# fabiocarrara/neural-ode-features

Measured on AMD Instinct MI355X. Metric: images/sec (fwd+adjoint) CIFAR-10 ODE-ResNet bs=128 at 1/2/4/8 GPU, higher is better.
Workload: dtype f32

## Files before the change

### neural-ode-features_amd/csrc/kernels_stem.hip

```cpp
#include "stem.h"

namespace node {

namespace {

typedef float f32x16 __attribute__((ext_vector_type(16)));
typedef __bf16 bf16x8 __attribute__((ext_vector_type(8)));
typedef __bf16 bf16x2 __attribute__((ext_vector_type(2)));
typedef float f32x2 __attribute__((ext_vector_type(2)));
typedef unsigned u32x4 __attribute__((ext_vector_type(4)));

__device__ __forceinline__ void split3(float x, bf16_t& h, bf16_t& m, bf16_t& l) {
  const __bf16 bh = (__bf16)x;
  const float r = x - (float)bh;
  const __bf16 bm = (__bf16)r;
  const float r2 = r - (float)bm;
  const __bf16 bl = (__bf16)r2;
  h = __builtin_bit_cast(bf16_t, bh);
  m = __builtin_bit_cast(bf16_t, bm);
  l = __builtin_bit_cast(bf16_t, bl);
}
__device__ __forceinline__ void split8(const float4& p, const float4& q, u32x4& hh, u32x4& mm, u32x4& ll) {
  const f32x2 v[4] = {{p.x, p.y}, {p.z, p.w}, {q.x, q.y}, {q.z, q.w}};
#pragma unroll
// ... 545 lines not shown
    if (a.dh) {
      *reinterpret_cast<float4*>(a.dh + o) = p0;
      *reinterpret_cast<float4*>(a.dh + o + 4) = p1;
    }
    if (a.dh3) {
      u32x4 hh, mm, ll;
      split8(p0, p1, hh, mm, ll);
      *reinterpret_cast<u32x4*>(a.dh3 + o) = hh;
      *reinterpret_cast<u32x4*>(a.dh3 + o + a.dh_plane) = mm;
      *reinterpret_cast<u32x4*>(a.dh3 + o + 2 * a.dh_plane) = ll;
    }
  }
}

__global__ __launch_bounds__(256) void k_stem_from_nchw(const float* __restrict__ src, float* __restrict__ dst, bf16_t* __restrict__ dst3,
                                                        size_t plane, int C, int HW) {
  __shared__ float tile[64][65];
  const int t = threadIdx.x;
  const int npb = (HW + 63) / 64, ncb = C / 64;
  const int n = blockIdx.x / (npb * ncb), rem = blockIdx.x - n * npb * ncb, cb = rem / npb, pb = rem - cb * npb;
  const int c0 = cb * 64, p0 = pb * 64;
  for (int idx = t; idx < 64 * 64; idx += 256) {
    const int cc = idx >> 6, pp = idx & 63;
    tile[cc][pp] = p0 + pp < HW ? src[((size_t)n * C + c0 + cc) * HW + p0 + pp] : 0.f;
  }
  __syncthreads();
  for (int idx = t; idx < 64 * 8; idx += 256) {
    const int pp = idx >> 3, q = idx & 7;
    if (p0 + pp >= HW) continue;
    float v[8];
#pragma unroll
    for (int k = 0; k < 8; ++k) v[k] = tile[8 * q + k][pp];
    const size_t o = ((size_t)n * HW + p0 + pp) * C + c0 + 8 * q;
    const float4 a0 = make_float4(v[0], v[1], v[2], v[3]), a1 = make_float4(v[4], v[5], v[6], v[7]);
    if (dst) {
      *reinterpret_cast<float4*>(dst + o) = a0;
      *reinterpret_cast<float4*>(dst + o + 4) = a1;
    }
    if (dst3) {
      u32x4 hh, mm, ll;
      split8(a0, a1, hh, mm, ll);
      *reinterpret_cast<u32x4*>(dst3 + o) = hh;
      *reinterpret_cast<u32x4*>(dst3 + o + plane) = mm;
      *reinterpret_cast<u32x4*>(dst3 + o + 2 * plane) = ll;
    }
  }
}

__global__ __launch_bounds__(256) void k_stem_split(const float* __restrict__ src, bf16_t* __restrict__ dst3, size_t plane, size_t n8) {
  const size_t i = (size_t)blockIdx.x * 256 + threadIdx.x;
  if (i >= n8) return;
  const float4 a0 = reinterpret_cast<const float4*>(src)[2 * i], a1 = reinterpret_cast<const float4*>(src)[2 * i + 1];
  u32x4 hh, mm, ll;
  split8(a0, a1, hh, mm, ll);
  *reinterpret_cast<u32x4*>(dst3 + 8 * i) = hh;
  *reinterpret_cast<u32x4*>(dst3 + 8 * i + plane) = mm;
  *reinterpret_cast<u32x4*>(dst3 + 8 * i + 2 * plane) = ll;
}

__global__ __launch_bounds__(256) void k_stem_to_nchw(const float* __restrict__ src, float* __restrict__ dst, int C, int HW) {
  __shared__ float tile[64][65];
  const int t = threadIdx.x;
  const int npb = (HW + 63) / 64, ncb = C / 64;
  const int n = blockIdx.x / (npb * ncb), rem = blockIdx.x - n * npb * ncb, cb = rem / npb, pb = rem - cb * npb;
  const int c0 = cb * 64, p0 = pb * 64;
// ... 23 lines not shown
    const float v = j.w[((size_t)co * j.Cin + ci) * j.taps + tap];
    bf16_t h, m, l;
    split3(v, h, m, l);
    const size_t of = ((size_t)tap * j.Cout + co) * j.Cin + ci, od = ((size_t)tap * j.Cin + ci) * j.Cout + co;
    j.wf[of] = h; j.wf[of + total] = m; j.wf[of + 2 * total] = l;
    j.wd[od] = h; j.wd[od + total] = m; j.wd[od + 2 * total] = l;
    return;
  }
  if (job == a.njobs) {
    if (a.w0t == nullptr || idx >= 28 * 64) return;
    const int k = (int)(idx / 64), co = (int)(idx % 64);
    a.w0t[idx] = k < a.k0 ? a.w0[co * a.k0 + k] : 0.f;
    return;
  }
  const int which = (int)(idx / 4096), e = (int)(idx % 4096);
  if (which >= a.nzero * 3) return;
  const int ten = which / 3, p = which - 3 * ten;
  if (e < a.zero_c[ten]) a.zero[ten][p * a.zero_plane[ten] + e] = 0;
}

__global__ __launch_bounds__(256) void k_stem_reduce(const SReduceArgs a) {
  __shared__ float part[4][64];
  int ji = 0;
  while (ji + 1 < a.njobs && blockIdx.x >= a.blk0[ji + 1]) ++ji;
  const SReduceJob& j = a.job[ji];
  const unsigned bx = blockIdx.x - a.blk0[ji];
  const int t = threadIdx.x;
  if (j.kind == 0) {
    const int co = bx / j.taps, tap = bx - co * j.taps;
    if (co >= j.Co) return;
// ... 107 lines not shown
}
void launch_stem_gn_bwd(const SGnArgs& a, hipStream_t s) {
  static bool attr[MAX_DEVICES] = {};
  allow_full_lds(reinterpret_cast<const void*>(k_stem_gn_bwd), attr);
  hipLaunchKernelGGL(k_stem_gn_bwd, dim3(a.N * (a.C / a.CB)), dim3(256), ((size_t)2 * a.HW * a.CB + 1024) * sizeof(float), s, a);
}

void launch_stem_prep(const SPrepArgs& a0, hipStream_t s) {
  SPrepArgs a = a0;
  unsigned at = 0;
  for (int i = 0; i < 6; ++i) {
    a.blk0[i] = at;
    if (i < a.njobs) at += (unsigned)(((size_t)a.job[i].taps * a.job[i].Cout * a.job[i].Cin + 255) / 256);
  }
  a.blk0[6] = at; at += (28 * 64 + 255) / 256;
  a.blk0[7] = at; at += (unsigned)(((size_t)a.nzero * 3 * 4096 + 255) / 256);
  a.blk0[8] = at;
  hipLaunchKernelGGL(k_stem_prep, dim3(at), dim3(256), 0, s, a);
}
void launch_stem_from_nchw(const float* src, float* dst_nhwc, bf16_t* dst3, size_t plane, int N, int C, int HW, hipStream_t s) {
  hipLaunchKernelGGL(k_stem_from_nchw, dim3(N * (C / 64) * ((HW + 63) / 64)), dim3(256), 0, s, src, dst_nhwc, dst3, plane, C, HW);
}
void launch_stem_split(const float* src, bf16_t* dst3, size_t plane, size_t n, hipStream_t s) {
  hipLaunchKernelGGL(k_stem_split, dim3((unsigned)((n / 8 + 255) / 256)), dim3(256), 0, s, src, dst3, plane, n / 8);
}
void launch_stem_to_nchw(const float* src_nhwc, float* dst, int N, int C, int HW, hipStream_t s) {
  hipLaunchKernelGGL(k_stem_to_nchw, dim3(N * (C / 64) * ((HW + 63) / 64)), dim3(256), 0, s, src_nhwc, dst, C, HW);
}
void launch_stem_reduce(const SReduceArgs& a0, hipStream_t s) {
  SReduceArgs a = a0;
  unsigned at = 0;
  for (int i = 0; i < a.njobs; ++i) {
    const SReduceJob& j = a.job[i];
    a.blk0[i] = at;
    at += (unsigned)(j.kind == 0 ? j.Co * j.taps : j.kind == 1 ? 64 : (2 * j.Co + 31) / 32);
  }
  a.blk0[a.njobs] = at;
  if (at == 0) return;
  hipLaunchKernelGGL(k_stem_reduce, dim3(at), dim3(256), 0, s, a);
// ... 4 lines not shown
```

### neural-ode-features_amd/csrc/kernels_w4.hip

```cpp
#include "wino4.h"
#include <cstdlib>
#include <cstring>

namespace node {

typedef float float16_t __attribute__((ext_vector_type(16)));
typedef __attribute__((address_space(3))) void* w4_lds_ptr_t;

#ifndef NODE_WT_STORES
#define NODE_WT_STORES 1
#endif
__device__ __forceinline__ void st_wt(float* p, float v) {
#if NODE_WT_STORES
  __hip_atomic_store(p, v, __ATOMIC_RELAXED, __HIP_MEMORY_SCOPE_AGENT);
#else
  *p = v;
#endif
}

__device__ __forceinline__ unsigned short w4_bf16_rne(float v) {
  const unsigned u = __builtin_bit_cast(unsigned, v);
  return (unsigned short)((u + 0x7FFFu + ((u >> 16) & 1u)) >> 16);
}
__device__ __forceinline__ float w4_bf16_f32(unsigned short b) { return __builtin_bit_cast(float, (unsigned)b << 16); }
// ... 1173 lines not shown
      }
      float* mrow = M + ((size_t)(rb * 8 + 2 * r4 + hi) * (gm.C >> 5) + 2 * ct + blk) * (36 * 128) + (size_t)scomp * 128 + l31;
      st_wt(mrow, s.x);
      st_wt(mrow + 32, s.y);
      st_wt(mrow + 64, s.z);
      st_wt(mrow + 96, s.w);
    }
  }
}



#endif

constexpr int W4SC_BLOCKS = 32;
__global__ __launch_bounds__(256) void k_w4_scales(W4ScaleJobs j, int nbig) {
  __shared__ float red[4];
  int job, part, parts;
  if ((int)blockIdx.x < nbig * W4SC_BLOCKS) {
    const int b = blockIdx.x / W4SC_BLOCKS;
    part = blockIdx.x - b * W4SC_BLOCKS; parts = W4SC_BLOCKS;
    job = j.bigjob[b];
  } else {
    job = 2 + ((int)blockIdx.x - nbig * W4SC_BLOCKS); part = 0; parts = 1;
  }
  const float* p = job < 2 ? j.w[job] : j.gb[job - 2];
  size_t n = job < 2 ? j.wn : (size_t)j.C;
  const bool big_vec = (job == 3 || job == 5) && j.vn[(job - 3) >> 1] != 0;
  if (big_vec) n = j.vn[(job - 3) >> 1];
  if (parts == 1 && big_vec) p = nullptr;
  float m = 0.f;
  if (p != nullptr) {
    const size_t i0 = (size_t)part * 256 + threadIdx.x, step = (size_t)parts * 256;
    if ((reinterpret_cast<uintptr_t>(p) & 15) == 0 && (n & 3) == 0) {
      const float4* q = reinterpret_cast<const float4*>(p);
      const size_t n4 = n >> 2;
      for (size_t i = i0; i < n4; i += 4 * step) {
        float4 v[4];
#pragma unroll
// ... 25 lines not shown
  }
  __hip_atomic_store(&sc->arrived, 0u, __ATOMIC_RELAXED, __HIP_MEMORY_SCOPE_AGENT);
  if (j.w[0] != nullptr) sc->e[W4_E_U1] = w4_scale_exp(3.49f * mx[0], 14);
  if (j.w[1] != nullptr) sc->e[W4_E_U2] = w4_scale_exp(3.49f * mx[1], 14);
  const float rm = sqrtf((float)j.gn_m);
  if (j.gb[0] != nullptr || j.gb[1] != nullptr) sc->e[W4_E_V1] = w4_scale_exp(49.f * (rm * mx[2] + mx[3]), 15);
  if (j.gb[2] != nullptr || j.gb[3] != nullptr) sc->e[W4_E_V2] = w4_scale_exp(49.f * (rm * mx[4] + mx[5]), 15);
}
void launch_w4_scales(const W4ScaleJobs& j_in, hipStream_t s) {
  W4ScaleJobs j = j_in;
  int nbig = 0;
  if (j.w[0] != nullptr) j.bigjob[nbig++] = 0;
  if (j.w[1] != nullptr) j.bigjob[nbig++] = 1;
  if (j.vn[0] != 0) j.bigjob[nbig++] = 3;
  if (j.vn[1] != 0) j.bigjob[nbig++] = 5;
  hipLaunchKernelGGL(k_w4_scales, dim3(nbig * W4SC_BLOCKS + 4), dim3(256), 0, s, j, nbig);
}

typedef _Float16 w4_f16x8 __attribute__((ext_vector_type(8)));
struct W4HStage { w4_u32x4 a[2][2], b[2][2]; };
struct W4HCursor { const w4_u32x4* a[2]; const w4_u32x4* b[2]; };
template <int NRB>
__device__ __forceinline__ void w4h_next(W4HStage& s, W4HCursor& cu) {
#pragma unroll
  for (int r = 0; r < NRB; ++r) {
    s.a[r][0] = cu.a[r][0];
    s.a[r][1] = cu.a[r][64];
    cu.a[r] += 128;
  }
#pragma unroll
  for (int c = 0; c < 2; ++c) {
// ... 1229 lines not shown
```

### neural-ode-features_amd/csrc/kernels_w4s.hip

```cpp
#include "wino4.h"
#include <cstring>

namespace node {

#ifndef W4S_THREADS_DEF
#define W4S_THREADS_DEF 128
#endif
constexpr int W4S_THREADS = W4S_THREADS_DEF;

#ifndef NODE_WT_STORES
#define NODE_WT_STORES 1
#endif
__device__ __forceinline__ void w4s_st_wt(float* p, float v) {
#if NODE_WT_STORES
  __hip_atomic_store(p, v, __ATOMIC_RELAXED, __HIP_MEMORY_SCOPE_AGENT);
#else
  *p = v;
#endif
}

template <int CTRL>
__device__ __forceinline__ float w4s_dpp(float v) {
  return __builtin_bit_cast(float, __builtin_amdgcn_update_dpp(0, __builtin_bit_cast(int, v), CTRL, 0xf, 0xf, true));
}
// ... 735 lines not shown
void launch_w4_input(const float* x_w4s, float* V, int N, int C, int Q, int Nv, hipStream_t s, const int* v_exp) {
  dim3 grid, block;
  w4s_grid(N, C, 1, Q, grid, block);
  if (Q == 1) hipLaunchKernelGGL(k_w4s_input<1>, grid, block, 0, s, x_w4s, V, C, Nv, v_exp);
  else hipLaunchKernelGGL(k_w4s_input<4>, grid, block, 0, s, x_w4s, V, C, Nv, v_exp);
}
void launch_w4_output(const float* M, float* y_w4s, int N, int C, int Q, hipStream_t s) {
  dim3 grid, block;
  w4s_grid(N, C, 1, Q, grid, block);
  if (Q == 1) hipLaunchKernelGGL(k_w4s_output<1>, grid, block, 0, s, M, y_w4s, C);
  else hipLaunchKernelGGL(k_w4s_output<4>, grid, block, 0, s, M, y_w4s, C);
}

__global__ __launch_bounds__(W4S_THREADS) void k_w4s_stem_in(const float* __restrict__ h, const float* __restrict__ gamma,
                                                             const float* __restrict__ beta, float eps, int cpg, float* __restrict__ xhat_s,
                                                             float* __restrict__ rstd, float* __restrict__ V, int C, int Nv) {
  W4Wave<1> wv;
  w4s_place(wv, C, nullptr, nullptr);
  const float* base = h + ((size_t)wv.n * 64 + (4 * wv.TY) * 8 + 4 * wv.TX) * C + wv.c;
  float y[4][4];
#pragma unroll
  for (int i = 0; i < 4; ++i)
#pragma unroll
    for (int j = 0; j < 4; ++j) y[i][j] = base[(size_t)(i * 8 + j) * C];
  float mean, rs;
  w4s_gn_stats(y, cpg, 1.0f / (float)(64 * cpg), eps, wv, mean, rs);
  const float gam = gamma[wv.c], bet = beta[wv.c];
  float xh[4][4], v[4][4];
#pragma unroll
  for (int i = 0; i < 4; ++i)
#pragma unroll
    for (int j = 0; j < 4; ++j) {
      xh[i][j] = (y[i][j] - mean) * rs;
      v[i][j] = fmaxf(fmaf(xh[i][j], gam, bet), 0.f);
    }
  const size_t f4 = ((size_t)wv.nv * (C >> 4) + wv.cb) * 256 + wv.lane;
#pragma unroll
  for (int i = 0; i < 4; ++i) w4s_st4(xhat_s, f4 + i * 64, xh[i]);
  if (wv.t == 0 && wv.c % cpg == 0) rstd[(size_t)wv.n * (C / cpg) + wv.c / cpg] = rs;
  w4s_put_v(v, wv, V, C, Nv);
}
__global__ __launch_bounds__(W4S_THREADS) void k_w4s_stem_out(const float* __restrict__ M, const float* __restrict__ res, float* __restrict__ out, int C) {
  W4Wave<1> wv;
  w4s_place(wv, C, nullptr, nullptr);
  float z[4][4];
  w4s_out_transform(w4s_m_ptr(M, wv, C), z);
  const float* rb = res + ((size_t)wv.n * 64 + (4 * wv.TY) * 8 + 4 * wv.TX) * C + wv.c;
  float* ob = out + ((size_t)wv.n * C + wv.c) * 64 + (4 * wv.TY) * 8 + 4 * wv.TX;
#pragma unroll
  for (int i = 0; i < 4; ++i) {
    float4 o;
    o.x = z[i][0] + rb[(size_t)(i * 8 + 0) * C];
    o.y = z[i][1] + rb[(size_t)(i * 8 + 1) * C];
    o.z = z[i][2] + rb[(size_t)(i * 8 + 2) * C];
    o.w = z[i][3] + rb[(size_t)(i * 8 + 3) * C];
    *reinterpret_cast<float4*>(ob + i * 8) = o;
  }
}
__global__ __launch_bounds__(W4S_THREADS) void k_w4s_stem_gin(const float* __restrict__ g, float* __restrict__ V, float* __restrict__ Z, int C, int Nv) {
  W4Wave<1> wv;
  w4s_place(wv, C, nullptr, nullptr);
  const float* gb = g + ((size_t)wv.n * C + wv.c) * 64 + (4 * wv.TY) * 8 + 4 * wv.TX;
  float v[4][4];
#pragma unroll
  for (int i = 0; i < 4; ++i) {
    const float4 q = *reinterpret_cast<const float4*>(gb + i * 8);
    v[i][0] = q.x; v[i][1] = q.y; v[i][2] = q.z; v[i][3] = q.w;
  }
  w4s_emit_z(v, wv.nv, Nv, C, wv.c, wv.t, Z);
  w4s_put_v(v, wv, V, C, Nv);
}
__global__ __launch_bounds__(256) void k_w4_du_to_dw(const float* __restrict__ dU, float* __restrict__ dW, int C) {
  const size_t CC = (size_t)C * C;
  const size_t idx = (size_t)blockIdx.x * 256 + threadIdx.x;
  if (idx >= CC) return;
  const int ci = (int)(idx / C), co = (int)(idx - (size_t)ci * C);
  float tq[6][3];
#pragma unroll
  for (int xi = 0; xi < 6; ++xi) {
    float u[6];
#pragma unroll
    for (int nu = 0; nu < 6; ++nu) u[nu] = dU[(size_t)(xi * 6 + nu) * CC + idx];
#pragma unroll
    for (int kw = 0; kw < 3; ++kw) {
      float sacc = 0.f;
// ... 8 lines not shown
  float* o = dW + ((size_t)co * C + ci) * 9;
#pragma unroll
  for (int kh = 0; kh < 3; ++kh)
#pragma unroll
    for (int kw = 0; kw < 3; ++kw) {
      float sacc = 0.f;
#pragma unroll
      for (int xi = 0; xi < 6; ++xi) {
        const float gq = (float)W4_G[xi][kh];
        if (gq != 0.f) sacc += gq * tq[xi][kw];
      }
      o[kh * 3 + kw] = sacc;
    }
}
void launch_w4s_stem_in(const float* h_nhwc, const float* gamma, const float* beta, float eps, int cpg, float* xhat_s, float* rstd, float* V,
                        int N, int C, int Nv, hipStream_t s) {
  dim3 grid, block;
  w4s_grid(N, C, cpg, 1, grid, block);
  hipLaunchKernelGGL(k_w4s_stem_in, grid, block, 0, s, h_nhwc, gamma, beta, eps, cpg, xhat_s, rstd, V, C, Nv);
}
void launch_w4s_stem_out(const float* M, const float* res_nhwc, float* out_nchw, int N, int C, hipStream_t s) {
  dim3 grid, block;
  w4s_grid(N, C, 1, 1, grid, block);
  hipLaunchKernelGGL(k_w4s_stem_out, grid, block, 0, s, M, res_nhwc, out_nchw, C);
}
void launch_w4s_stem_gin(const float* g_nchw, float* V, float* Z, int N, int C, int Nv, hipStream_t s) {
  dim3 grid, block;
  w4s_grid(N, C, 1, 1, grid, block);
  hipLaunchKernelGGL(k_w4s_stem_gin, grid, block, 0, s, g_nchw, V, Z, C, Nv);
}
void launch_w4_du_to_dw(const float* dU, float* dW, int C, hipStream_t s) {
  const size_t CC = (size_t)C * C;
  hipLaunchKernelGGL(k_w4_du_to_dw, dim3((unsigned)((CC + 255) / 256)), dim3(256), 0, s, dU, dW, C);
}

}
```

### neural-ode-features_amd/csrc/stem.h

```cpp
#pragma once
#include "node_internal.h"

namespace node {

typedef unsigned short bf16_t;

struct SConvArgs {
  const bf16_t* in;
  size_t in_plane;
  int zero_row;
  const bf16_t* w;
  size_t w_plane;
  float* out;
  const float* res;
  const float* bias;
  int accumulate;
  const bf16_t* w2;
  size_t w2_plane;
  float* out2;
  const bf16_t* in2;
  int N, IH, IW;
  int OH, OW;
  int Cin, Cout;
  int KH, KW, sshift, pad;
// ... 39 lines not shown
  size_t dh_plane;
  float* gpart;
  int N, HW, C, cpg, CB;
  float eps;
};
int stem_gn_cb(int HW, int C, int cpg);
void launch_stem_gn_fwd(const SGnArgs& a, hipStream_t s);
void launch_stem_gn_bwd(const SGnArgs& a, hipStream_t s);

struct SPrepJob { const float* w; bf16_t* wf; bf16_t* wd; int Cout, Cin, taps; };
struct SPrepArgs {
  SPrepJob job[6];
  int njobs;
  const float* w0; float* w0t; int k0;
  bf16_t* zero[10]; size_t zero_plane[10]; int zero_c[10]; int nzero;
  unsigned blk0[9];
};
void launch_stem_prep(const SPrepArgs& a, hipStream_t s);
void launch_stem_from_nchw(const float* src, float* dst_nhwc, bf16_t* dst3, size_t plane, int N, int C, int HW, hipStream_t s);
void launch_stem_to_nchw(const float* src_nhwc, float* dst, int N, int C, int HW, hipStream_t s);
void launch_stem_split(const float* src, bf16_t* dst3, size_t plane, size_t n , hipStream_t s);
struct SReduceJob { const float* slab; float* out; float* out2; int kind, ns, Co, Ci, taps; };
struct SReduceArgs { SReduceJob job[12]; int njobs; unsigned blk0[13]; };
void launch_stem_reduce(const SReduceArgs& a, hipStream_t s);

}
```

### neural-ode-features_amd/csrc/stem_api.hip

```cpp
#include "stem.h"
#include "wino4.h"
#include "../../include/node_hip.h"
#include <cstdarg>
#include <cstdio>
#include <cstring>

using namespace node;

namespace {

int failf(int code, const char* fmt, ...) {
  char buf[512];
  va_list ap;
  va_start(ap, fmt);
  vsnprintf(buf, sizeof(buf), fmt, ap);
  va_end(ap);
  return set_error(code, buf);
}

struct Bump {
  char* base;
  size_t off;
  explicit Bump(void* b) : base((char*)b), off(0) {}
  template <typename T>
// ... 56 lines not shown
struct StemPlan {
  int N, Cin0, H, W, F;
  int H0, W0, H1, W1, H2, W2, R0, R1, R2;
  float eps;
  float* w0t;
  Filt c1, c2, d1, c3, c4, d2;
  float *h0, *h1, *s1, *x1, *h3, *s2, *outn;
  Trip a0, a1, a2, a3;
  float* stats[4];
  float *da3, *da2, *da1, *da0, *dh0;
  Trip g3, dh3t, dx1t, dh1t;
  float* gpart[4];
  Wg w4, w3, w2, w1, w0;
  bool f4;
  bool f4_b16;
  float *xh4, *rs4, *Va, *Vg, *M4, *Z4, *dU4, *U4[2], *dh3n;
  unsigned short* Ub4[2];
  size_t bytes;
};

bool stem_takes_w4(const node_stem_shape* sh) {
  const char* e = getenv("NODE_TUNE_STEM_W4");
  if (e && atoi(e) == 0) return false;
  const int h2 = ((sh->h - 2 - 1) / 2 + 1 - 1) / 2 + 1, w2 = ((sh->w - 2 - 1) / 2 + 1 - 1) / 2 + 1;
  return h2 == 8 && w2 == 8 && sh->filters % 128 == 0 && sh->n % 8 == 0 && 16 % (sh->filters / 32) == 0;
}

StemPlan make_stem_plan(const node_stem_shape* sh, void* base) {
  StemPlan p;
  memset(&p, 0, sizeof(p));
  p.N = sh->n; p.Cin0 = sh->in_ch; p.H = sh->h; p.W = sh->w; p.F = sh->filters; p.eps = sh->eps;
  p.H0 = p.H - 2; p.W0 = p.W - 2;
  p.H1 = down2(p.H0); p.W1 = down2(p.W0);
  p.H2 = down2(p.H1); p.W2 = down2(p.W1);
  p.R0 = p.N * p.H0 * p.W0; p.R1 = p.N * p.H1 * p.W1; p.R2 = p.N * p.H2 * p.W2;
  const int F = p.F, G64 = 32, GF = F < 32 ? F : 32;
  Bump b(base);
  p.w0t = b.take<float>(28 * 64);
  p.c1 = take_filt(b, 64, 64, 9);
  p.c2 = take_filt(b, 64, 64, 9);
// ... 35 lines not shown
  p.w1 = take_wg(b, p.R1, 64, 64, 9, true);
  {
    int ns = p.R0 / 256;
    if (ns > 1024) ns = 1024;
    if (ns < 1) ns = 1;
    int rps = ((p.R0 + ns - 1) / ns + 7) & ~7;
    p.w0.rps = rps;
    p.w0.nsplit = (p.R0 + rps - 1) / rps;
    p.w0.slab = b.take<float>((size_t)p.w0.nsplit * 64 * 32);
    p.w0.slab2 = nullptr;
  }
  p.f4 = stem_takes_w4(sh);
  if (p.f4) {
    const int Nv = p.N;
    p.f4_b16 = w4_uses_bf16(Nv, F);
    p.xh4 = b.take<float>((size_t)p.R2 * F);
    p.rs4 = b.take<float>((size_t)p.N * GF);
    p.Va = b.take<float>(w4_v_elems(Nv, F));
    p.Vg = b.take<float>(w4_v_elems(Nv, F));
    p.M4 = b.take<float>(w4_v_elems(Nv, F));
    p.Z4 = b.take<float>(w4_z_elems(Nv, F));
    p.dU4 = b.take<float>((size_t)W4_COMPS * F * F);
    for (int i = 0; i < 2; ++i) {
      p.U4[i] = b.take<float>(w4_u_elems(F));
      p.Ub4[i] = b.take<unsigned short>(w4_ub_elems(F));
    }
    p.dh3n = b.take<float>((size_t)p.R2 * F);
  }
  p.bytes = b.off + 256;
  return p;
}

int check_stem_shape(const node_stem_shape* sh) {
  if (!sh) return failf(NODE_ERR_NULL, "shape is NULL");
  if (sh->n <= 0 || sh->in_ch <= 0 || sh->h < 5 || sh->w < 5 || sh->filters <= 0) return failf(NODE_ERR_SHAPE, "bad stem shape");
  if (sh->in_ch > 3) return failf(NODE_ERR_UNSUPPORTED, "the stem's first layer takes in_ch <= 3 (got %d)", sh->in_ch);
  if (sh->filters % 64 != 0) return failf(NODE_ERR_UNSUPPORTED, "the stem's kernels take filters %% 64 == 0 (got %d)", sh->filters);
  const size_t biggest = (size_t)sh->n * (sh->h - 2) * (sh->w - 2) * 64;
  if (biggest >= ((size_t)1 << 31)) return failf(NODE_ERR_UNSUPPORTED, "stem tensors must stay under 2^31 elements");
  if (stem_gn_cb((sh->h - 2) * (sh->w - 2), 64, 2) == 0)
    return failf(NODE_ERR_UNSUPPORTED, "the stem's GroupNorm passes hold (sample, 8 channels) blocks in LDS: images up to %d pixels "
                 "behind the first layer (got %d x %d)", 150 * 1024 / 64, sh->h - 2, sh->w - 2);
// ... 105 lines not shown
  if (rc != NODE_OK) return rc;
  if (!prm || !x || !out || !ws) return failf(NODE_ERR_NULL, "a required pointer is NULL");
  const float* const* pp = reinterpret_cast<const float* const*>(prm);
  for (int i = 0; i < 16; ++i)
    if (!pp[i]) return failf(NODE_ERR_NULL, "stem parameter %d is NULL", i);
  if (((uintptr_t)ws) & 255) return failf(NODE_ERR_ARG, "workspace must be 256-byte aligned");
  StemPlan p = make_stem_plan(shape, ws);
  if (ws_bytes < p.bytes) return failf(NODE_ERR_WORKSPACE, "stem workspace too small: %zu < %zu", ws_bytes, p.bytes);
  hipStream_t st = (hipStream_t)stream;
  const int N = p.N, F = p.F;

  SPrepArgs pa;
  memset(&pa, 0, sizeof(pa));
  const Filt* fl[6] = {&p.c1, &p.c2, &p.d1, &p.c3, &p.c4, &p.d2};
  const float* fw[6] = {prm->b1_c1_w, prm->b1_c2_w, prm->b1_ds_w, prm->b2_c1_w, prm->b2_c2_w, prm->b2_ds_w};
  for (int i = 0; i < 6; ++i) pa.job[i] = {fw[i], fl[i]->wf, fl[i]->wd, fl[i]->Cout, fl[i]->Cin, fl[i]->taps};
  pa.njobs = 6;
  pa.w0 = prm->conv0_w; pa.w0t = p.w0t; pa.k0 = 9 * p.Cin0;
  const Trip* tz[8] = {&p.a0, &p.a1, &p.a2, &p.a3, &p.g3, &p.dh3t, &p.dx1t, &p.dh1t};
  for (int i = 0; i < 8; ++i) {
    pa.zero[i] = tz[i]->p + (size_t)tz[i]->rows * tz[i]->C;
    pa.zero_plane[i] = tz[i]->plane;
    pa.zero_c[i] = tz[i]->C;
  }
  pa.nzero = 8;
  if (F > 4096) return failf(NODE_ERR_UNSUPPORTED, "filters > 4096");
  launch_stem_prep(pa, st);
  if ((rc = launch_ok("stem_prep")) != NODE_OK) return rc;

  launch_stem_conv0_fwd(x, p.w0t, prm->conv0_b, p.h0, N, p.Cin0, p.H, p.W, st);
  if ((rc = launch_ok("stem_conv0_fwd")) != NODE_OK) return rc;
  {
// ... 21 lines not shown
    if ((rc = launch_ok("stem_conv")) != NODE_OK) return rc;
  }
  {
    SGnArgs g = gn_args(p.x1, prm->b2_n1_w, prm->b2_n1_b, p.stats[2], N, p.H1 * p.W1, 64, p.eps);
    g.a3 = p.a2.p; g.a_plane = p.a2.plane;
    launch_stem_gn_fwd(g, st);
    if ((rc = launch_ok("stem_gn_fwd")) != NODE_OK) return rc;
  }
  {
    SConvArgs c = conv_fwd_args(p.a2, p.c3, p.h3, N, p.H1, p.W1, p.H2, p.W2, 3, 2, 1);
    c.w2 = p.d2.wf; c.w2_plane = p.d2.plane; c.out2 = p.s2;
    launch_stem_conv(c, st);
    if ((rc = launch_ok("stem_conv")) != NODE_OK) return rc;
  }
  if (p.f4) {
    W4PackJobs jobs;
    memset(&jobs, 0, sizeof(jobs));
    for (int i = 0; i < 2; ++i) {
      jobs.w[i] = prm->b2_c2_w; jobs.u[i] = p.U4[i]; jobs.ub[i] = p.f4_b16 ? p.Ub4[i] : nullptr; jobs.dgrad[i] = i; jobs.plain[i] = 1;
    }
    launch_w4_pack(jobs, 2, F, st);
    if ((rc = launch_ok("w4_pack")) != NODE_OK) return rc;
    launch_w4s_stem_in(p.h3, prm->b2_n2_w, prm->b2_n2_b, p.eps, F / 32, p.xh4, p.rs4, p.Va, N, F, N, st);
    if ((rc = launch_ok("w4s_stem_in")) != NODE_OK) return rc;
    launch_w4_gemm(p.Va, p.U4[0], p.M4, nullptr, N, F, st, p.f4_b16 ? p.Ub4[0] : nullptr);
    if ((rc = launch_ok("w4_gemm")) != NODE_OK) return rc;
    launch_w4s_stem_out(p.M4, p.s2, out, N, F, st);
    return launch_ok("node_stem_fwd");
  }
  {
    SGnArgs g = gn_args(p.h3, prm->b2_n2_w, prm->b2_n2_b, p.stats[3], N, p.H2 * p.W2, F, p.eps);
    g.a3 = p.a3.p; g.a_plane = p.a3.plane;
    launch_stem_gn_fwd(g, st);
    if ((rc = launch_ok("stem_gn_fwd")) != NODE_OK) return rc;
  }
  {
    SConvArgs c = conv_fwd_args(p.a3, p.c4, p.outn, N, p.H2, p.W2, p.H2, p.W2, 3, 1, 1);
    c.res = p.s2;
    launch_stem_conv(c, st);
    if ((rc = launch_ok("stem_conv")) != NODE_OK) return rc;
// ... 8 lines not shown
  w4_refresh_tuning();
  int rc = check_stem_shape(shape);
  if (rc != NODE_OK) return rc;
  if (!prm || !x || !grad_out || !gr || !ws) return failf(NODE_ERR_NULL, "a required pointer is NULL");
  const float* const* pp = reinterpret_cast<const float* const*>(prm);
  float* const* gp = reinterpret_cast<float* const*>(gr);
  for (int i = 0; i < 16; ++i)
    if (!pp[i] || !gp[i]) return failf(NODE_ERR_NULL, "stem parameter / gradient %d is NULL", i);
  if (((uintptr_t)ws) & 255) return failf(NODE_ERR_ARG, "workspace must be 256-byte aligned");
  StemPlan p = make_stem_plan(shape, ws);
  if (ws_bytes < p.bytes) return failf(NODE_ERR_WORKSPACE, "stem workspace too small: %zu < %zu", ws_bytes, p.bytes);
  hipStream_t st = (hipStream_t)stream;
  const int N = p.N, F = p.F;
  const int HW0 = p.H0 * p.W0, HW1 = p.H1 * p.W1, HW2 = p.H2 * p.W2;

  launch_stem_from_nchw(grad_out, nullptr, p.g3.p, p.g3.plane, N, F, HW2, st);
  if ((rc = launch_ok("stem_from_nchw")) != NODE_OK) return rc;
  if (p.f4) {
    launch_w4s_stem_gin(grad_out, p.Vg, p.Z4, N, F, N, st);
    if ((rc = launch_ok("w4s_stem_gin")) != NODE_OK) return rc;
    launch_w4_gemm(p.Vg, p.U4[1], p.M4, nullptr, N, F, st, p.f4_b16 ? p.Ub4[1] : nullptr);
    if ((rc = launch_ok("w4_gemm")) != NODE_OK) return rc;
    W4sArgs a;
    memset(&a, 0, sizeof(a));
    a.N = N; a.Q = 1; a.Nv = N; a.C = F; a.cpg = F / 32; a.eps = p.eps;
    a.h.M = p.M4; a.h.gamma = prm->b2_n2_w; a.h.beta = prm->b2_n2_b; a.h.xhat_s = p.xh4; a.h.rstd = p.rs4; a.h.osign = 1.f;
    a.h.gpart = p.gpart[3]; a.h.out_nhwc = p.dh3n;
    launch_w4s_pass(2, 0, a, st);
    if ((rc = launch_ok("w4s_pass")) != NODE_OK) return rc;
    launch_stem_split(p.dh3n, p.dh3t.p, p.dh3t.plane, (size_t)p.R2 * F, st);
    if ((rc = launch_ok("stem_split")) != NODE_OK) return rc;
    W4WgradArgs wa;
    memset(&wa, 0, sizeof(wa));
    wa.V1 = p.Va; wa.Z1 = p.Z4; wa.dU = p.dU4; wa.N = N; wa.C = F;
    launch_w4_wgrad(wa, st);
    if ((rc = launch_ok("w4_wgrad")) != NODE_OK) return rc;
    launch_w4_du_to_dw(p.dU4, gr->b2_c2_w, F, st);
    if ((rc = launch_ok("w4_du_to_dw")) != NODE_OK) return rc;
  } else {
    launch_stem_wgrad(wgrad_args(p.g3, nullptr, p.a3, p.w4, N, p.H2, p.W2, p.H2, p.W2, F, F, 3, 1, 1), st);
    if ((rc = launch_ok("stem_wgrad")) != NODE_OK) return rc;
    launch_stem_conv(conv_dgrad_args(p.g3, p.c4, p.da3, N, p.H2, p.W2, p.H2, p.W2, 3, 1, 1), st);
    if ((rc = launch_ok("stem_conv")) != NODE_OK) return rc;
    {
      SGnArgs g = gn_args(p.h3, prm->b2_n2_w, prm->b2_n2_b, p.stats[3], N, HW2, F, p.eps);
      g.da = p.da3; g.dh = nullptr; g.dh3 = p.dh3t.p; g.dh_plane = p.dh3t.plane; g.gpart = p.gpart[3];
      launch_stem_gn_bwd(g, st);
      if ((rc = launch_ok("stem_gn_bwd")) != NODE_OK) return rc;
    }
  }
// ... 146 lines not shown
```

### neural-ode-features_amd/csrc/wino4.h

```cpp
#pragma once
#include "node_internal.h"

namespace node {

constexpr int W4_COMPS = 36;

__device__ constexpr float W4_BT[6][6] = {{1.f, -1.5f, -2.f, 1.5f, 1.f, 0.f}, {0.f, -1.f, 0.5f, 2.5f, 1.f, 0.f},
                                          {0.f, 1.f, -2.5f, 0.5f, 1.f, 0.f},  {0.f, -2.f, -1.f, 2.f, 1.f, 0.f},
                                          {0.f, 0.5f, -1.f, -0.5f, 1.f, 0.f}, {0.f, 1.f, -1.5f, -2.f, 1.5f, 1.f}};
__device__ constexpr float W4_AT[4][6] = {{1.f, 1.f, 1.f, 1.f, 1.f, 0.f},
                                          {0.f, 1.f, -1.f, 0.5f, -2.f, 0.f},
                                          {0.f, 1.f, 1.f, 0.25f, 4.f, 0.f},
                                          {0.f, 1.f, -1.f, 0.125f, -8.f, 1.f}};
__device__ constexpr double W4_G[6][3] = {{1.0, 0.0, 0.0},
                                          {1.0 / 3, 1.0 / 3, 1.0 / 3},
                                          {-1.0 / 3, 1.0 / 3, -1.0 / 3},
                                          {-16.0 / 15, -8.0 / 15, -4.0 / 15},
                                          {1.0 / 15, -2.0 / 15, 4.0 / 15},
                                          {0.0, 0.0, 1.0}};

struct W4Geom {
  int N, C, RB, G8, R;
};
__host__ __device__ inline W4Geom w4_geom(int N, int C) {
// ... 37 lines not shown
    __hip_atomic_store(&sc->ovf, 0u, __ATOMIC_RELAXED, __HIP_MEMORY_SCOPE_AGENT);
    if (g > 0.f && g < INFINITY) sc->e[4] = w4_scale_exp(g, W4_G_TOP);
    if (ovf) sc->n_retry += 1;
  }
  return ovf;
}
void launch_w4_gscale(W4Scales* sc, hipStream_t s, int skew = 0);
constexpr int W4_E_U1 = 0, W4_E_U2 = 1, W4_E_V1 = 2, W4_E_V2 = 3, W4_E_G = 4;
struct W4ScaleJobs {
  const float* w[2];
  size_t wn;
  const float* gb[4];
  size_t vn[2];
  int C, gn_m;
  W4Scales* sc;
  int bigjob[4];
};
void launch_w4_scales(const W4ScaleJobs& j, hipStream_t s);
constexpr int W4_SLACK = 16 * 256;
__host__ __device__ inline size_t w4_v_elems(int N, int C) { return (size_t)W4_COMPS * 4 * N * C + W4_SLACK; }
__host__ __device__ inline size_t w4_u_elems(int C) { return (size_t)W4_COMPS * C * C + W4_SLACK; }

struct W4sHead {
  const float* M;
  const float* bias;
  const float* tmapS;
  EvalTime et;
  const float* gamma;
  const float* beta;
  float osign;
// ... 57 lines not shown

constexpr float W4_MIN_TOL = 0.99e-5f;
struct W4PackJobs { const float* w[4]; float* u[4]; unsigned short* ub[4]; int dgrad[4]; int plain[4]; unsigned* uh[4]; const int* uh_exp[4]; };
bool w4_uses_bf16(int N, int C);
__host__ __device__ inline size_t w4_ub_elems(int C) { return (size_t)W4_COMPS * C * C * 3 + 8 * 1536; }
void launch_w4_pack(const W4PackJobs& jobs, int count, int C, hipStream_t s);
void launch_w4_gemm(const float* V, const float* U, float* M, const Ctrl* ctrl, int N, int C, hipStream_t s,
                    const unsigned short* Ub = nullptr);
bool w4_f16_fits(int N, int C);
void launch_w4_gemm_f16(const unsigned* Vh, const unsigned* Uh, float* M, const Ctrl* ctrl, int N, int C, const int* v_exp, const int* u_exp,
                        hipStream_t s);
void launch_w4_split_check(const float* x, float* out, size_t n, hipStream_t s);
void launch_w4_input(const float* x_w4s, float* V, int N, int C, int Q, int Nv, hipStream_t s, const int* v_exp = nullptr);
void launch_w4_output(const float* M, float* y_w4s, int N, int C, int Q, hipStream_t s);
void launch_w4s_stem_in(const float* h_nhwc, const float* gamma, const float* beta, float eps, int cpg, float* xhat_s, float* rstd, float* V,
                        int N, int C, int Nv, hipStream_t s);
void launch_w4s_stem_out(const float* M, const float* res_nhwc, float* out_nchw, int N, int C, hipStream_t s);
void launch_w4s_stem_gin(const float* g_nchw, float* V, float* Z, int N, int C, int Nv, hipStream_t s);
void launch_w4_du_to_dw(const float* dU, float* dW, int C, hipStream_t s);

}
```

Measured before the change: 27920.

## Run stem Winograd-4 conv in scaled fp16 with fused gradient max tracking

Switches the stem's F(4,3) Winograd GEMMs (forward, dgrad and wgrad) to the scaled fp16 path when shapes fit, enabled by default through an env switch. Per-tensor exponents come from a scales kernel for weights and GN parameters. The gradient's absolute max is gathered with atomics inside the existing NCHW-to-NHWC transpose, so no extra pass over the data is needed. The c4 weight split is also dropped from the prep job when Winograd is used. This aims to cut GEMM time and memory traffic, at the cost of an extra scales launch, atomics, and fp16 range and accuracy risk.

```diff
diff --git a/neural-ode-features_amd/csrc/kernels_stem.hip b/neural-ode-features_amd/csrc/kernels_stem.hip
--- a/neural-ode-features_amd/csrc/kernels_stem.hip
+++ b/neural-ode-features_amd/csrc/kernels_stem.hip
@@ -583,17 +583,30 @@
 }
 
 __global__ __launch_bounds__(256) void k_stem_from_nchw(const float* __restrict__ src, float* __restrict__ dst, bf16_t* __restrict__ dst3,
-                                                        size_t plane, int C, int HW) {
+                                                        size_t plane, int C, int HW, unsigned* __restrict__ gmax, int nslots) {
   __shared__ float tile[64][65];
+  __shared__ float red[4];
   const int t = threadIdx.x;
   const int npb = (HW + 63) / 64, ncb = C / 64;
   const int n = blockIdx.x / (npb * ncb), rem = blockIdx.x - n * npb * ncb, cb = rem / npb, pb = rem - cb * npb;
   const int c0 = cb * 64, p0 = pb * 64;
+  float m = 0.f;
   for (int idx = t; idx < 64 * 64; idx += 256) {
     const int cc = idx >> 6, pp = idx & 63;
-    tile[cc][pp] = p0 + pp < HW ? src[((size_t)n * C + c0 + cc) * HW + p0 + pp] : 0.f;
-  }
-  __syncthreads();
+    const float v = p0 + pp < HW ? src[((size_t)n * C + c0 + cc) * HW + p0 + pp] : 0.f;
+    tile[cc][pp] = v;
+    const float av = fabsf(v);
+    m = av < INFINITY ? fmaxf(m, av) : m;
+  }
+  if (gmax != nullptr) {
+    for (int o = 32; o > 0; o >>= 1) m = fmaxf(m, __shfl_xor(m, o, 64));
+    if ((t & 63) == 0) red[t >> 6] = m;
+  }
+  __syncthreads();
+  if (gmax != nullptr && t == 0) {
+    m = fmaxf(fmaxf(red[0], red[1]), fmaxf(red[2], red[3]));
+    if (m > 0.f) atomicMax(&gmax[blockIdx.x % nslots], __builtin_bit_cast(unsigned, m));
+  }
   for (int idx = t; idx < 64 * 8; idx += 256) {
     const int pp = idx >> 3, q = idx & 7;
     if (p0 + pp >= HW) continue;
@@ -616,8 +629,10 @@
   }
 }
 
-__global__ __launch_bounds__(256) void k_stem_split(const float* __restrict__ src, bf16_t* __restrict__ dst3, size_t plane, size_t n8) {
+__global__ __launch_bounds__(256) void k_stem_split(const float* __restrict__ src, bf16_t* __restrict__ dst3, size_t plane, size_t n8,
+                                                    unsigned* __restrict__ clr, int nclr) {
   const size_t i = (size_t)blockIdx.x * 256 + threadIdx.x;
+  if (clr != nullptr && blockIdx.x == 0 && (int)threadIdx.x < nclr) clr[threadIdx.x] = 0u;
   if (i >= n8) return;
   const float4 a0 = reinterpret_cast<const float4*>(src)[2 * i], a1 = reinterpret_cast<const float4*>(src)[2 * i + 1];
   u32x4 hh, mm, ll;
@@ -671,6 +686,7 @@
     return;
   }
   const int which = (int)(idx / 4096), e = (int)(idx % 4096);
+  if (which == a.nzero * 3 && e < a.nzw) a.zw[e] = 0u;
   if (which >= a.nzero * 3) return;
   const int ten = which / 3, p = which - 3 * ten;
   if (e < a.zero_c[ten]) a.zero[ten][p * a.zero_plane[ten] + e] = 0;
@@ -808,15 +824,17 @@
     if (i < a.njobs) at += (unsigned)(((size_t)a.job[i].taps * a.job[i].Cout * a.job[i].Cin + 255) / 256);
   }
   a.blk0[6] = at; at += (28 * 64 + 255) / 256;
-  a.blk0[7] = at; at += (unsigned)(((size_t)a.nzero * 3 * 4096 + 255) / 256);
+  a.blk0[7] = at; at += (unsigned)(((size_t)(a.nzero * 3 + (a.nzw > 0 ? 1 : 0)) * 4096 + 255) / 256);
   a.blk0[8] = at;
   hipLaunchKernelGGL(k_stem_prep, dim3(at), dim3(256), 0, s, a);
 }
-void launch_stem_from_nchw(const float* src, float* dst_nhwc, bf16_t* dst3, size_t plane, int N, int C, int HW, hipStream_t s) {
-  hipLaunchKernelGGL(k_stem_from_nchw, dim3(N * (C / 64) * ((HW + 63) / 64)), dim3(256), 0, s, src, dst_nhwc, dst3, plane, C, HW);
-}
-void launch_stem_split(const float* src, bf16_t* dst3, size_t plane, size_t n, hipStream_t s) {
-  hipLaunchKernelGGL(k_stem_split, dim3((unsigned)((n / 8 + 255) / 256)), dim3(256), 0, s, src, dst3, plane, n / 8);
+void launch_stem_from_nchw(const float* src, float* dst_nhwc, bf16_t* dst3, size_t plane, int N, int C, int HW, hipStream_t s,
+                           unsigned* gmax, int nslots) {
+  hipLaunchKernelGGL(k_stem_from_nchw, dim3(N * (C / 64) * ((HW + 63) / 64)), dim3(256), 0, s, src, dst_nhwc, dst3, plane, C, HW, gmax,
+                     nslots);
+}
+void launch_stem_split(const float* src, bf16_t* dst3, size_t plane, size_t n, hipStream_t s, unsigned* clr, int nclr) {
+  hipLaunchKernelGGL(k_stem_split, dim3((unsigned)((n / 8 + 255) / 256)), dim3(256), 0, s, src, dst3, plane, n / 8, clr, nclr);
 }
 void launch_stem_to_nchw(const float* src_nhwc, float* dst, int N, int C, int HW, hipStream_t s) {
   hipLaunchKernelGGL(k_stem_to_nchw, dim3(N * (C / 64) * ((HW + 63) / 64)), dim3(256), 0, s, src_nhwc, dst, C, HW);
diff --git a/neural-ode-features_amd/csrc/kernels_w4.hip b/neural-ode-features_amd/csrc/kernels_w4.hip
--- a/neural-ode-features_amd/csrc/kernels_w4.hip
+++ b/neural-ode-features_amd/csrc/kernels_w4.hip
@@ -1211,15 +1211,15 @@
 #endif
 
 constexpr int W4SC_BLOCKS = 32;
-__global__ __launch_bounds__(256) void k_w4_scales(W4ScaleJobs j, int nbig) {
+__global__ __launch_bounds__(256) void k_w4_scales(W4ScaleJobs j, int nbig, int bpj) {
   __shared__ float red[4];
   int job, part, parts;
-  if ((int)blockIdx.x < nbig * W4SC_BLOCKS) {
-    const int b = blockIdx.x / W4SC_BLOCKS;
-    part = blockIdx.x - b * W4SC_BLOCKS; parts = W4SC_BLOCKS;
+  if ((int)blockIdx.x < nbig * bpj) {
+    const int b = blockIdx.x / bpj;
+    part = blockIdx.x - b * bpj; parts = bpj;
     job = j.bigjob[b];
   } else {
-    job = 2 + ((int)blockIdx.x - nbig * W4SC_BLOCKS); part = 0; parts = 1;
+    job = 2 + ((int)blockIdx.x - nbig * bpj); part = 0; parts = 1;
   }
   const float* p = job < 2 ? j.w[job] : j.gb[job - 2];
   size_t n = job < 2 ? j.wn : (size_t)j.C;
@@ -1275,7 +1275,8 @@
   if (j.w[1] != nullptr) j.bigjob[nbig++] = 1;
   if (j.vn[0] != 0) j.bigjob[nbig++] = 3;
   if (j.vn[1] != 0) j.bigjob[nbig++] = 5;
-  hipLaunchKernelGGL(k_w4_scales, dim3(nbig * W4SC_BLOCKS + 4), dim3(256), 0, s, j, nbig);
+  const int bpj = j.blocks > 0 ? j.blocks : W4SC_BLOCKS;
+  hipLaunchKernelGGL(k_w4_scales, dim3(nbig * bpj + 4), dim3(256), 0, s, j, nbig, bpj);
 }
 
 typedef _Float16 w4_f16x8 __attribute__((ext_vector_type(8)));
diff --git a/neural-ode-features_amd/csrc/kernels_w4s.hip b/neural-ode-features_amd/csrc/kernels_w4s.hip
--- a/neural-ode-features_amd/csrc/kernels_w4s.hip
+++ b/neural-ode-features_amd/csrc/kernels_w4s.hip
@@ -773,7 +773,8 @@
 
 __global__ __launch_bounds__(W4S_THREADS) void k_w4s_stem_in(const float* __restrict__ h, const float* __restrict__ gamma,
                                                              const float* __restrict__ beta, float eps, int cpg, float* __restrict__ xhat_s,
-                                                             float* __restrict__ rstd, float* __restrict__ V, int C, int Nv) {
+                                                             float* __restrict__ rstd, float* __restrict__ V, int C, int Nv,
+                                                             const int* v_exp) {
   W4Wave<1> wv;
   w4s_place(wv, C, nullptr, nullptr);
   const float* base = h + ((size_t)wv.n * 64 + (4 * wv.TY) * 8 + 4 * wv.TX) * C + wv.c;
@@ -797,7 +798,7 @@
 #pragma unroll
   for (int i = 0; i < 4; ++i) w4s_st4(xhat_s, f4 + i * 64, xh[i]);
   if (wv.t == 0 && wv.c % cpg == 0) rstd[(size_t)wv.n * (C / cpg) + wv.c / cpg] = rs;
-  w4s_put_v(v, wv, V, C, Nv);
+  w4s_put_v(v, wv, V, C, Nv, v_exp);
 }
 __global__ __launch_bounds__(W4S_THREADS) void k_w4s_stem_out(const float* __restrict__ M, const float* __restrict__ res, float* __restrict__ out, int C) {
   W4Wave<1> wv;
@@ -816,7 +817,8 @@
     *reinterpret_cast<float4*>(ob + i * 8) = o;
   }
 }
-__global__ __launch_bounds__(W4S_THREADS) void k_w4s_stem_gin(const float* __restrict__ g, float* __restrict__ V, float* __restrict__ Z, int C, int Nv) {
+__global__ __launch_bounds__(W4S_THREADS) void k_w4s_stem_gin(const float* __restrict__ g, float* __restrict__ V, float* __restrict__ Z, int C, int Nv,
+                                                              const unsigned* __restrict__ gmax, int* __restrict__ e_out) {
   W4Wave<1> wv;
   w4s_place(wv, C, nullptr, nullptr);
   const float* gb = g + ((size_t)wv.n * C + wv.c) * 64 + (4 * wv.TY) * 8 + 4 * wv.TX;
@@ -826,8 +828,20 @@
     const float4 q = *reinterpret_cast<const float4*>(gb + i * 8);
     v[i][0] = q.x; v[i][1] = q.y; v[i][2] = q.z; v[i][3] = q.w;
   }
-  w4s_emit_z(v, wv.nv, Nv, C, wv.c, wv.t, Z);
-  w4s_put_v(v, wv, V, C, Nv);
+  if (gmax == nullptr) {
+    w4s_emit_z(v, wv.nv, Nv, C, wv.c, wv.t, Z);
+    w4s_put_v(v, wv, V, C, Nv);
+    return;
+  }
+  static_assert(W4S_STEM_GSLOTS == 64, "one slot per lane");
+  float m = __builtin_bit_cast(float, gmax[threadIdx.x & 63]);
+  for (int o = 32; o > 0; o >>= 1) m = fmaxf(m, __shfl_xor(m, o, 64));
+  const int e = w4_scale_exp(m, W4S_STEM_G_TOP);
+  if (blockIdx.x == 0 && blockIdx.y == 0 && threadIdx.x == 0) *e_out = e;
+  const float ps = ldexpf(1.f, e);
+  const bool odd = (wv.c15 & 1) != 0;
+  w4s_emit_zh(v, w4s_vh_ptr(Z, wv, C), (size_t)4 * Nv * C, ps, odd);
+  w4s_emit_v(v, wv.ty, wv.tx, w4s_vh_ptr(V, wv, C), (size_t)4 * Nv * C, ps, odd);
 }
 __global__ __launch_bounds__(256) void k_w4_du_to_dw(const float* __restrict__ dU, float* __restrict__ dW, int C) {
   const size_t CC = (size_t)C * C;
@@ -866,20 +880,20 @@
     }
 }
 void launch_w4s_stem_in(const float* h_nhwc, const float* gamma, const float* beta, float eps, int cpg, float* xhat_s, float* rstd, float* V,
-                        int N, int C, int Nv, hipStream_t s) {
+                        int N, int C, int Nv, hipStream_t s, const int* v_exp) {
   dim3 grid, block;
   w4s_grid(N, C, cpg, 1, grid, block);
-  hipLaunchKernelGGL(k_w4s_stem_in, grid, block, 0, s, h_nhwc, gamma, beta, eps, cpg, xhat_s, rstd, V, C, Nv);
+  hipLaunchKernelGGL(k_w4s_stem_in, grid, block, 0, s, h_nhwc, gamma, beta, eps, cpg, xhat_s, rstd, V, C, Nv, v_exp);
 }
 void launch_w4s_stem_out(const float* M, const float* res_nhwc, float* out_nchw, int N, int C, hipStream_t s) {
   dim3 grid, block;
   w4s_grid(N, C, 1, 1, grid, block);
   hipLaunchKernelGGL(k_w4s_stem_out, grid, block, 0, s, M, res_nhwc, out_nchw, C);
 }
-void launch_w4s_stem_gin(const float* g_nchw, float* V, float* Z, int N, int C, int Nv, hipStream_t s) {
+void launch_w4s_stem_gin(const float* g_nchw, float* V, float* Z, int N, int C, int Nv, hipStream_t s, const unsigned* gmax, int* e_out) {
   dim3 grid, block;
   w4s_grid(N, C, 1, 1, grid, block);
-  hipLaunchKernelGGL(k_w4s_stem_gin, grid, block, 0, s, g_nchw, V, Z, C, Nv);
+  hipLaunchKernelGGL(k_w4s_stem_gin, grid, block, 0, s, g_nchw, V, Z, C, Nv, gmax, e_out);
 }
 void launch_w4_du_to_dw(const float* dU, float* dW, int C, hipStream_t s) {
   const size_t CC = (size_t)C * C;
diff --git a/neural-ode-features_amd/csrc/stem.h b/neural-ode-features_amd/csrc/stem.h
--- a/neural-ode-features_amd/csrc/stem.h
+++ b/neural-ode-features_amd/csrc/stem.h
@@ -77,12 +77,15 @@
   int njobs;
   const float* w0; float* w0t; int k0;
   bf16_t* zero[10]; size_t zero_plane[10]; int zero_c[10]; int nzero;
+  unsigned* zw; int nzw;
   unsigned blk0[9];
 };
 void launch_stem_prep(const SPrepArgs& a, hipStream_t s);
-void launch_stem_from_nchw(const float* src, float* dst_nhwc, bf16_t* dst3, size_t plane, int N, int C, int HW, hipStream_t s);
+void launch_stem_from_nchw(const float* src, float* dst_nhwc, bf16_t* dst3, size_t plane, int N, int C, int HW, hipStream_t s,
+                           unsigned* gmax = nullptr, int nslots = 1);
 void launch_stem_to_nchw(const float* src_nhwc, float* dst, int N, int C, int HW, hipStream_t s);
-void launch_stem_split(const float* src, bf16_t* dst3, size_t plane, size_t n , hipStream_t s);
+void launch_stem_split(const float* src, bf16_t* dst3, size_t plane, size_t n , hipStream_t s, unsigned* clr = nullptr,
+                       int nclr = 0);
 struct SReduceJob { const float* slab; float* out; float* out2; int kind, ns, Co, Ci, taps; };
 struct SReduceArgs { SReduceJob job[12]; int njobs; unsigned blk0[13]; };
 void launch_stem_reduce(const SReduceArgs& a, hipStream_t s);
diff --git a/neural-ode-features_amd/csrc/stem_api.hip b/neural-ode-features_amd/csrc/stem_api.hip
--- a/neural-ode-features_amd/csrc/stem_api.hip
+++ b/neural-ode-features_amd/csrc/stem_api.hip
@@ -2,6 +2,7 @@
 #include "wino4.h"
 #include "../../include/node_hip.h"
 #include <cstdarg>
+#include <cstddef>
 #include <cstdio>
 #include <cstring>
 
@@ -94,8 +95,10 @@
   Wg w4, w3, w2, w1, w0;
   bool f4;
   bool f4_b16;
+  bool f4_h;
   float *xh4, *rs4, *Va, *Vg, *M4, *Z4, *dU4, *U4[2], *dh3n;
   unsigned short* Ub4[2];
+  W4Scales* sc4;
   size_t bytes;
 };
 
@@ -104,6 +107,10 @@
   if (e && atoi(e) == 0) return false;
   const int h2 = ((sh->h - 2 - 1) / 2 + 1 - 1) / 2 + 1, w2 = ((sh->w - 2 - 1) / 2 + 1 - 1) / 2 + 1;
   return h2 == 8 && w2 == 8 && sh->filters % 128 == 0 && sh->n % 8 == 0 && 16 % (sh->filters / 32) == 0;
+}
+bool stem_takes_f16() {
+  const char* e = getenv("NODE_TUNE_STEM_F16");
+  return !(e && atoi(e) == 0);
 }
 
 StemPlan make_stem_plan(const node_stem_shape* sh, void* base) {
@@ -169,18 +176,20 @@
   if (p.f4) {
     const int Nv = p.N;
     p.f4_b16 = w4_uses_bf16(Nv, F);
+    p.f4_h = p.f4_b16 && stem_takes_f16() && w4_f16_fits(Nv, F) && w4_wgrad_f16_fits(Nv, F);
     p.xh4 = b.take<float>((size_t)p.R2 * F);
     p.rs4 = b.take<float>((size_t)p.N * GF);
     p.Va = b.take<float>(w4_v_elems(Nv, F));
     p.Vg = b.take<float>(w4_v_elems(Nv, F));
     p.M4 = b.take<float>(w4_v_elems(Nv, F));
-    p.Z4 = b.take<float>(w4_z_elems(Nv, F));
+    p.Z4 = b.take<float>(w4_v_elems(Nv, F));
     p.dU4 = b.take<float>((size_t)W4_COMPS * F * F);
     for (int i = 0; i < 2; ++i) {
       p.U4[i] = b.take<float>(w4_u_elems(F));
       p.Ub4[i] = b.take<unsigned short>(w4_ub_elems(F));
     }
     p.dh3n = b.take<float>((size_t)p.R2 * F);
+    p.sc4 = b.take<W4Scales>(1);
   }
   p.bytes = b.off + 256;
   return p;
@@ -316,8 +325,15 @@
   memset(&pa, 0, sizeof(pa));
   const Filt* fl[6] = {&p.c1, &p.c2, &p.d1, &p.c3, &p.c4, &p.d2};
   const float* fw[6] = {prm->b1_c1_w, prm->b1_c2_w, prm->b1_ds_w, prm->b2_c1_w, prm->b2_c2_w, prm->b2_ds_w};
-  for (int i = 0; i < 6; ++i) pa.job[i] = {fw[i], fl[i]->wf, fl[i]->wd, fl[i]->Cout, fl[i]->Cin, fl[i]->taps};
-  pa.njobs = 6;
+  int nj = 0;
+  for (int i = 0; i < 6; ++i)
+    if (!(p.f4 && fl[i] == &p.c4))
+      pa.job[nj++] = {fw[i], fl[i]->wf, fl[i]->wd, fl[i]->Cout, fl[i]->Cin, fl[i]->taps};
+  pa.njobs = nj;
+  if (p.f4) {
+    pa.zw = reinterpret_cast<unsigned*>(p.sc4);
+    pa.nzw = (int)(offsetof(W4Scales, gmax) / sizeof(unsigned)) + W4S_STEM_GSLOTS;
+  }
   pa.w0 = prm->conv0_w; pa.w0t = p.w0t; pa.k0 = 9 * p.Cin0;
   const Trip* tz[8] = {&p.a0, &p.a1, &p.a2, &p.a3, &p.g3, &p.dh3t, &p.dx1t, &p.dh1t};
   for (int i = 0; i < 8; ++i) {
@@ -369,16 +385,32 @@
     if ((rc = launch_ok("stem_conv")) != NODE_OK) return rc;
   }
   if (p.f4) {
+    int* const e = p.sc4->e;
+    if (p.f4_h) {
+      W4ScaleJobs sj;
+      memset(&sj, 0, sizeof(sj));
+      sj.w[0] = prm->b2_c2_w; sj.wn = (size_t)F * F * 9;
+      sj.gb[0] = prm->b2_n2_w; sj.gb[1] = prm->b2_n2_b;
+      sj.C = F; sj.gn_m = (F / 32) * 64; sj.sc = p.sc4;
+      sj.blocks = 256;
+      launch_w4_scales(sj, st);
+      if ((rc = launch_ok("w4_scales")) != NODE_OK) return rc;
+    }
     W4PackJobs jobs;
     memset(&jobs, 0, sizeof(jobs));
     for (int i = 0; i < 2; ++i) {
-      jobs.w[i] = prm->b2_c2_w; jobs.u[i] = p.U4[i]; jobs.ub[i] = p.f4_b16 ? p.Ub4[i] : nullptr; jobs.dgrad[i] = i; jobs.plain[i] = 1;
+      jobs.w[i] = prm->b2_c2_w; jobs.u[i] = p.U4[i]; jobs.ub[i] = (p.f4_b16 && !p.f4_h) ? p.Ub4[i] : nullptr; jobs.dgrad[i] = i; jobs.plain[i] = 1;
+      if (p.f4_h) { jobs.uh[i] = reinterpret_cast<unsigned*>(p.U4[i]); jobs.uh_exp[i] = &e[W4_E_U1]; }
     }
     launch_w4_pack(jobs, 2, F, st);
     if ((rc = launch_ok("w4_pack")) != NODE_OK) return rc;
-    launch_w4s_stem_in(p.h3, prm->b2_n2_w, prm->b2_n2_b, p.eps, F / 32, p.xh4, p.rs4, p.Va, N, F, N, st);
+    launch_w4s_stem_in(p.h3, prm->b2_n2_w, prm->b2_n2_b, p.eps, F / 32, p.xh4, p.rs4, p.Va, N, F, N, st, p.f4_h ? &e[W4_E_V1] : nullptr);
     if ((rc = launch_ok("w4s_stem_in")) != NODE_OK) return rc;
-    launch_w4_gemm(p.Va, p.U4[0], p.M4, nullptr, N, F, st, p.f4_b16 ? p.Ub4[0] : nullptr);
+    if (p.f4_h)
+      launch_w4_gemm_f16(reinterpret_cast<const unsigned*>(p.Va), reinterpret_cast<const unsigned*>(p.U4[0]), p.M4, nullptr, N, F, &e[W4_E_V1],
+                         &e[W4_E_U1], st);
+    else
+      launch_w4_gemm(p.Va, p.U4[0], p.M4, nullptr, N, F, st, p.f4_b16 ? p.Ub4[0] : nullptr);
     if ((rc = launch_ok("w4_gemm")) != NODE_OK) return rc;
     launch_w4s_stem_out(p.M4, p.s2, out, N, F, st);
     return launch_ok("node_stem_fwd");
@@ -417,12 +449,17 @@
   const int N = p.N, F = p.F;
   const int HW0 = p.H0 * p.W0, HW1 = p.H1 * p.W1, HW2 = p.H2 * p.W2;
 
-  launch_stem_from_nchw(grad_out, nullptr, p.g3.p, p.g3.plane, N, F, HW2, st);
+  launch_stem_from_nchw(grad_out, nullptr, p.g3.p, p.g3.plane, N, F, HW2, st, p.f4_h ? p.sc4->gmax : nullptr, W4S_STEM_GSLOTS);
   if ((rc = launch_ok("stem_from_nchw")) != NODE_OK) return rc;
   if (p.f4) {
-    launch_w4s_stem_gin(grad_out, p.Vg, p.Z4, N, F, N, st);
+    int* const e = p.sc4->e;
+    launch_w4s_stem_gin(grad_out, p.Vg, p.Z4, N, F, N, st, p.f4_h ? p.sc4->gmax : nullptr, p.f4_h ? &e[W4_E_G] : nullptr);
     if ((rc = launch_ok("w4s_stem_gin")) != NODE_OK) return rc;
-    launch_w4_gemm(p.Vg, p.U4[1], p.M4, nullptr, N, F, st, p.f4_b16 ? p.Ub4[1] : nullptr);
+    if (p.f4_h)
+      launch_w4_gemm_f16(reinterpret_cast<const unsigned*>(p.Vg), reinterpret_cast<const unsigned*>(p.U4[1]), p.M4, nullptr, N, F, &e[W4_E_G],
+                         &e[W4_E_U1], st);
+    else
+      launch_w4_gemm(p.Vg, p.U4[1], p.M4, nullptr, N, F, st, p.f4_b16 ? p.Ub4[1] : nullptr);
     if ((rc = launch_ok("w4_gemm")) != NODE_OK) return rc;
     W4sArgs a;
     memset(&a, 0, sizeof(a));
@@ -431,12 +468,17 @@
     a.h.gpart = p.gpart[3]; a.h.out_nhwc = p.dh3n;
     launch_w4s_pass(2, 0, a, st);
     if ((rc = launch_ok("w4s_pass")) != NODE_OK) return rc;
-    launch_stem_split(p.dh3n, p.dh3t.p, p.dh3t.plane, (size_t)p.R2 * F, st);
+    launch_stem_split(p.dh3n, p.dh3t.p, p.dh3t.plane, (size_t)p.R2 * F, st, p.f4_h ? p.sc4->gmax : nullptr, W4S_STEM_GSLOTS);
     if ((rc = launch_ok("stem_split")) != NODE_OK) return rc;
-    W4WgradArgs wa;
-    memset(&wa, 0, sizeof(wa));
-    wa.V1 = p.Va; wa.Z1 = p.Z4; wa.dU = p.dU4; wa.N = N; wa.C = F;
-    launch_w4_wgrad(wa, st);
+    if (p.f4_h) {
+      launch_w4_wgrad_f16(reinterpret_cast<const unsigned*>(p.Va), reinterpret_cast<const unsigned*>(p.Z4), nullptr, nullptr, p.dU4, nullptr, N, F,
+                          &e[W4_E_V1], nullptr, &e[W4_E_G], st);
+    } else {
+      W4WgradArgs wa;
+      memset(&wa, 0, sizeof(wa));
+      wa.V1 = p.Va; wa.Z1 = p.Z4; wa.dU = p.dU4; wa.N = N; wa.C = F;
+      launch_w4_wgrad(wa, st);
+    }
     if ((rc = launch_ok("w4_wgrad")) != NODE_OK) return rc;
     launch_w4_du_to_dw(p.dU4, gr->b2_c2_w, F, st);
     if ((rc = launch_ok("w4_du_to_dw")) != NODE_OK) return rc;
diff --git a/neural-ode-features_amd/csrc/wino4.h b/neural-ode-features_amd/csrc/wino4.h
--- a/neural-ode-features_amd/csrc/wino4.h
+++ b/neural-ode-features_amd/csrc/wino4.h
@@ -75,6 +75,7 @@
   size_t vn[2];
   int C, gn_m;
   W4Scales* sc;
+  int blocks;
   int bigjob[4];
 };
 void launch_w4_scales(const W4ScaleJobs& j, hipStream_t s);
@@ -162,9 +163,12 @@
 void launch_w4_input(const float* x_w4s, float* V, int N, int C, int Q, int Nv, hipStream_t s, const int* v_exp = nullptr);
 void launch_w4_output(const float* M, float* y_w4s, int N, int C, int Q, hipStream_t s);
 void launch_w4s_stem_in(const float* h_nhwc, const float* gamma, const float* beta, float eps, int cpg, float* xhat_s, float* rstd, float* V,
-                        int N, int C, int Nv, hipStream_t s);
+                        int N, int C, int Nv, hipStream_t s, const int* v_exp = nullptr);
 void launch_w4s_stem_out(const float* M, const float* res_nhwc, float* out_nchw, int N, int C, hipStream_t s);
-void launch_w4s_stem_gin(const float* g_nchw, float* V, float* Z, int N, int C, int Nv, hipStream_t s);
+constexpr int W4S_STEM_GSLOTS = 64;
+constexpr int W4S_STEM_G_TOP = 7;
+void launch_w4s_stem_gin(const float* g_nchw, float* V, float* Z, int N, int C, int Nv, hipStream_t s, const unsigned* gmax = nullptr,
+                         int* e_out = nullptr);
 void launch_w4_du_to_dw(const float* dU, float* dW, int C, hipStream_t s);
 
 }
```

Result: no change. 27870 (median of 3 runs) (-0.2%).
